# QueensGambit/CrazyAra

Hardware: AMD Instinct MI355X
Metric: nn_evals_per_sec (higher is better)
Workload: dtype f16x3; 1 GPU; crazyhouse RISEv2 19-block (34x8x8 planes -> 5184 policy + value), batch=256, inputs resident in HBM, random-init seeded weights; batch=256, parallelism=replicas x1, precision=float16x3

## Files before the change

crazyara_amd/_capi.py:

```python
from __future__ import annotations

import ctypes as C
import os

_HERE = os.path.dirname(os.path.abspath(__file__))
LIB_PATH = os.path.join(_HERE, "lib", "libcrazyara_hip.so")

c_float_p = C.POINTER(C.c_float)
c_int_p = C.POINTER(C.c_int)

SIGNATURES = {
    "mi_last_error": (C.c_char_p, []),
    "mi_version": (C.c_char_p, []),
    "mi_device_count": (C.c_int, []),
    "mi_host_alloc": (C.c_void_p, [C.c_size_t]),
    "mi_host_free": (None, [C.c_void_p]),
    "mi_net_create": (C.c_void_p, [C.c_char_p, C.c_int, C.c_int, C.c_char_p]),
    "mi_net_destroy": (None, [C.c_void_p]),
    "mi_net_calibrate_int8": (C.c_int, [C.c_char_p, C.c_int, C.c_void_p, C.c_int]),
    "mi_net_has_int8_calibration": (C.c_int, [C.c_char_p]),
    "mi_onnx_to_cranet": (C.c_int, [C.c_char_p, C.c_char_p]),
    "mi_e4m3_from_float": (C.c_int, [C.c_float]),
    "mi_e5m2_from_float": (C.c_int, [C.c_float]),
    "mi_net_design": (C.c_int, [C.c_void_p, c_int_p, c_int_p, c_int_p, c_int_p, c_int_p]),
# ... 1 lines not shown
    "mi_net_flops_per_position": (C.c_double, [C.c_void_p]),
    "mi_net_predict": (C.c_int, [C.c_void_p, C.c_void_p, C.c_void_p, C.c_void_p, C.c_void_p]),
    "mi_net_submit": (C.c_int, [C.c_void_p, C.c_void_p, C.c_void_p, C.c_void_p, C.c_void_p]),
    "mi_net_last_submit_zero_copy": (C.c_int, [C.c_void_p]),
    "mi_net_wait": (C.c_int, [C.c_void_p]),
    "mi_net_device_buffers": (C.c_int, [C.c_void_p] + [C.POINTER(C.c_void_p)] * 5),
    "mi_net_keep_logits": (C.c_int, [C.c_void_p, C.c_int]),
    "mi_net_block_dump": (C.c_void_p, [C.c_void_p, c_int_p]),
    "mi_net_forward_device": (C.c_int, [C.c_void_p]),
    "mi_net_sync": (C.c_int, [C.c_void_p]),
    "mi_net_stream": (C.c_void_p, [C.c_void_p]),
    "mi_net_time_forward": (C.c_int, [C.c_void_p, C.c_int, c_float_p]),
    "mi_net_op_count": (C.c_int, [C.c_void_p]),
    "mi_net_time_ops": (C.c_int, [C.c_void_p, C.c_int, C.POINTER(C.c_char_p), c_float_p]),
    "mi_net_op_kernel": (C.c_char_p, [C.c_void_p, C.c_int]),
    "mi_net_submit_boards": (C.c_int, [C.c_void_p, C.c_void_p, C.c_int, C.c_int, C.c_void_p, C.c_void_p, C.c_void_p]),
    "mi_net_submit_boards_gathered": (C.c_int, [C.c_void_p, C.c_void_p, C.c_int, C.c_int, C.c_void_p, C.c_void_p, C.c_uint, C.c_void_p,
                                                C.c_void_p, C.c_void_p]),
    "mi_net_create_experts": (C.c_void_p, [C.c_char_p, C.c_int, C.c_int, C.c_char_p, C.c_int]),
    "mi_net_num_experts": (C.c_int, [C.c_void_p]),
    "mi_expert_dirs": (C.c_int, [C.c_char_p, C.c_int, C.c_int, C.c_char_p, C.c_int]),
    "mi_net_set_expert_routing": (C.c_int, [C.c_void_p, C.c_int]),
    "mi_net_submit_boards_phases": (C.c_int, [C.c_void_p, C.c_void_p, C.c_int, c_int_p]),
    "mi_net_predict_routed": (C.c_int, [C.c_void_p, C.c_void_p, C.c_void_p, C.c_void_p, C.c_void_p, C.c_void_p]),
    "mi_desc_game_phase": (C.c_int, [C.c_void_p, C.c_int, C.c_int]),
    "mi_pos_create": (C.c_void_p, [C.c_char_p, C.c_int, C.c_char_p]),
    "mi_pos_clone": (C.c_void_p, [C.c_void_p]),
    "mi_pos_destroy": (None, [C.c_void_p]),
    "mi_pos_fen": (C.c_int, [C.c_void_p, C.c_char_p, C.c_int]),
    "mi_pos_side_to_move": (C.c_int, [C.c_void_p]),
# ... 100 lines not shown
```

crazyara_amd/csrc/capi.cpp:

```cpp
#include "../../include/crazyara_hip.h"

#include <hip/hip_runtime.h>

#include <exception>
#include <stdexcept>
#include <string>

#include "capi_common.h"
#include "nn/onnx_import.h"
#include "nn/rise_net.h"

namespace {
thread_local std::string g_err;
template <typename F> int guard(F&& f) { return cra_guard(static_cast<F&&>(f)); }
}

void cra_set_error(const std::string& msg) { g_err = msg; }
const char* cra_get_error() { return g_err.c_str(); }

#include "capi_net.h"

namespace {
cra::RiseNet& plain_net(const mi_net* net, const char* what, const char* why = nullptr) {
    if (!net->plain)
// ... 193 lines not shown
    return guard([&] { net->any->wait(); });
}
void* mi_net_stream(mi_net* net) { return net ? static_cast<void*>(net->any->stream()) : nullptr; }

int mi_net_time_forward(mi_net* net, int iters, float* ms_total) {
    if (!net || !ms_total) { g_err = "null argument"; return 1; }
    return guard([&] { *ms_total = plain_net(net, "a device-resident forward").time_forward(iters); });
}
int mi_net_op_count(const mi_net* net) { return net && net->plain ? net->plain->launches_per_forward() : 0; }
const char* mi_net_op_kernel(const mi_net* net, int op) {
    if (!net || !net->plain || op < 0 || op >= net->plain->launches_per_forward()) { g_err = "mi_net_op_kernel: no such op"; return nullptr; }
    const char* name = nullptr;
    if (guard([&] { name = net->plain->op_kernel(op); })) return nullptr;
    return name;
}
int mi_net_time_ops(mi_net* net, int iters, const char** names, float* ms) {
    if (!net || !ms) { g_err = "null argument"; return 1; }
    return guard([&] {
        cra::RiseNet& plain = plain_net(net, "per-op timing");
        const int n = plain.launches_per_forward();
        for (int i = 0; i < n; ++i) {
            if (names) names[i] = plain.op_name(i);
            ms[i] = 0.f;
        }
        plain.time_ops(iters, ms);
    });
}

}
```

crazyara_amd/csrc/nn/kernels.h:

```cpp
#pragma once
#include <hip/hip_runtime.h>
#include <cstdint>

namespace cra {

typedef _Float16 half_t;

constexpr int kSquares = 64;

inline int64_t packed_weight_elems(int cout_pad, int k_total) { return int64_t(cout_pad) * k_total; }

struct ConvArgs {
    const void* x;
    const void* wpk;
    const void* wpk_lo;
    const float* bias;
    const void* resid;
    void* out;
    int batch;
    int cin;
    int cout_pad;
    int cout_real;
    int cout_ld;
    int ks;
// ... 51 lines not shown
    float w1_inv, w3_scale, w3_inv;
    int tail;
};
static_assert(sizeof(X3TowerBlock) == 96, "the tower kernels index a device array of these");
struct X3TowerArgs {
    const float* x;
    float* y;
    const X3TowerBlock* blocks;
    int nblocks;
    int batch;
    int p8;
    int ks;
    int symmetric;
    int no_tail;
    int no_quad;
};
void launch_tower_x3(const X3TowerArgs& a, hipStream_t s);
const char* tower_x3_kernel_name(const X3TowerArgs& a);
void launch_tower_x3_tail(const X3TowerArgs& a, hipStream_t s);
void init_x3_tail_kernel_attributes();
void launch_tower_x3_quad(const X3TowerArgs& a, hipStream_t s);
void init_x3_quad_kernel_attributes();
bool block_x3w_supports(int C, int ks);
void launch_block_x3w(const BlockArgs& a, hipStream_t s);
void init_x3_wblock_kernel_attributes();
void launch_se_gate_w(const float* pool, float* gate, int kind, const float* w1t, const float* w2t, const float* b1, int batch, int C, hipStream_t s);
constexpr int kX3WSplitMaxG = 8;
struct X3WSplitArgs {
    BlockArgs blk;
    const float* x_parts;
    float* y_parts;
    int gin, G;
    int stream_in;
};
int x3w_split_chunks(int cop_pad);
int x3w_split_shares(int cop_pad, int boards, int cu_count);
void launch_block_x3w_split(const X3WSplitArgs& a, hipStream_t s);
// ... 225 lines not shown
```

crazyara_amd/csrc/nn/precision.cpp:

```cpp
#include <cstdlib>
#include <stdexcept>

#include "rise_net.h"

namespace cra {

namespace {
constexpr bool kX3ValueHeadOneLaunch = true;
}

RiseNet::DevSwitches::DevSwitches() {
    if (const char* e = getenv("CRA_X3_CONV_DEV")) conv_dev = atoi(e);
    device_graph = getenv("CRA_DEVICE_GRAPH") != nullptr;
    lane_graph = getenv("CRA_LANE_GRAPH") != nullptr;
    lane_no_graph = getenv("CRA_LANE_NO_GRAPH") != nullptr;
    predict_copy = getenv("CRA_PREDICT_COPY") != nullptr;
    predict_zero_copy = getenv("CRA_PREDICT_ZERO_COPY") != nullptr;
    if (const char* e = getenv("CRA_LANE_LAUNCHES")) lane_launches = e[0];
    lane_sync = getenv("CRA_LANE_SYNC") != nullptr;
    if (const char* e = getenv("CRA_X3_TOWER")) x3_symmetric = e[0] == 's';
    if (const char* e = getenv("CRA_X3_SPLIT_DEV")) x3_split_dev = atoi(e);
    no_small_path = getenv("CRA_NO_SMALL_PATH") != nullptr;
    if (const char* e = getenv("CRA_SMALL_BATCH_CONV_SPLIT")) small_conv_split = atoi(e);
    tower_trace = getenv("CRA_TOWER_TRACE") != nullptr;
    x3_value_one_launch = kX3ValueHeadOneLaunch;
    if (const char* e = getenv("CRA_X3_VALUE_HEAD")) x3_value_one_launch = e[0] == 'o';
    value_head_debug = getenv("CRA_VALUE_HEAD_DEBUG") != nullptr;
    if (const char* e = getenv("CRA_VALUE_HEAD_LDS_PAD")) value_head_lds_pad = atoi(e);
    if (const char* e = getenv("CRA_VALUE_HEAD_VARIANT")) value_head_variant = atoi(e);
    x3_no_head_chain = getenv("CRA_X3_NO_HEAD_CHAIN") != nullptr;
    x3_no_tail = getenv("CRA_X3_NO_TAIL") != nullptr;
    x3_no_quad = getenv("CRA_X3_NO_QUAD") != nullptr;
    small_batch_heads_apart = getenv("CRA_SMALL_BATCH_HEADS_APART") != nullptr;
}

Precision parse_precision(const std::string& precision) {
    Precision v;
    std::string prec = precision;
    auto strip = [&](const std::string& tag) {
        if (prec.size() <= tag.size() || prec.compare(prec.size() - tag.size(), tag.size(), tag) != 0) return false;
        prec.resize(prec.size() - tag.size());
        return true;
    };
    if (strip("-3k")) v.one_launch = false;
    if (strip("-8w")) v.thin_waves = true;
    if (strip("-1wg")) v.board_split = false;
    if (strip("-1b")) v.boards_per_wg = 1;
// ... 33 lines not shown
```

crazyara_amd/csrc/nn/rise_net.h:

```cpp
#pragma once
#include <hip/hip_runtime.h>
#include <memory>
#include <string>
#include <utility>
#include <vector>

#include "board_net.h"
#include "netfile.h"

namespace cra {

uint8_t float_to_e4m3(float v);
uint8_t float_to_e5m2(float v);

struct Precision {
    enum class Mode { Float32, Float16, Float16x3, Float16p8, Fp8, Int8 };
    Mode mode = Mode::Float16;
    bool fused = true;
    bool tower = true;
    bool one_launch = true;
    bool thin_waves = false;
    bool board_split = true;
    bool wblock = false;
    bool wnet = false;
// ... 41 lines not shown
    void run_group(const Group& g);

    std::vector<std::pair<float, float>> calibration_maxima(const float* planes_host, int n_boards);

    void keep_logits(bool on) override;
    void* enable_block_dump(int* n_tiles);
    void dev_launch_op(int op, int iters);
    float* value_head_debug() const { return value_head_dbg_; }
    int dev_screen_prepare();
    long dev_screen_run(int op, int launches, long* words);
    std::string dev_screen_info(int op) const;
    void forward_async();

    int launches_per_forward() const { return launches_; }
    const char* op_name(int i) const;
    const char* op_kernel(int i) const;
    void time_ops(int iters, float* ms);
    float time_forward(int iters);

    struct IoOverride {
        const float* planes = nullptr;
        float* value = nullptr;
        float* probs = nullptr;
        float* aux = nullptr;
    };
    bool last_submit_was_zero_copy() const { return last_zero_copy_; }

private:
    friend class ExpertSet;
    struct ForwardCall {
// ... 23 lines not shown
        bool predict_copy = false;
        bool predict_zero_copy = false;
        char lane_launches = 0;
        bool lane_sync = false;
        bool x3_symmetric = false;
        int x3_split_dev = 0;
        bool no_small_path = false;
        int small_conv_split = 2;
        bool tower_trace = false;
        bool x3_value_one_launch;
        bool value_head_debug = false;
        int value_head_lds_pad = -1;
        int value_head_variant = 0;
        bool x3_no_head_chain = false;
        bool x3_no_tail = false;
        bool x3_no_quad = false;
        bool small_batch_heads_apart = false;
        DevSwitches();
    } dev_;
    float* value_head_dbg_ = nullptr;

    std::string model_file_path_;
    Precision prec_;
    std::vector<std::pair<float, float>> int8_calib_;
    static constexpr int kBoardSplitMaxBatch = 64;
    std::unique_ptr<RiseNet> small_;
    bool owns_stream_ = true;
    int stream_slot_ = -1;
    std::string precision_arg_;
    int cu_count_ = 256;
// ... 14 lines not shown
```

crazyara_amd/csrc/nn/rise_net.hip:

```cpp
#include "rise_net.h"

#include <cmath>
#include <cstdio>
#include <cstring>
#include <fstream>
#include <algorithm>

#include "net_streams.h"
#include "onnx_import.h"
#include "rise_net_impl.h"
#include "../chess/planes_host.h"

namespace cra {

RiseNet::RiseNet(const std::string& model_path, int device_id, int batch_size, const std::string& precision, const RiseNet* parent)
    : BoardNet(device_id), impl_(new Impl) {
    if (batch_size <= 0) throw std::invalid_argument("batch size must be positive");
    precision_arg_ = precision;
    prec_ = parse_precision(precision);
    design_.batch = batch_size;

    std::string dir, file;
    auto ends_with = [&](const char* ext) { const size_t n = strlen(ext); return model_path.size() > n && model_path.compare(model_path.size() - n, n, ext) == 0; };
    if (ends_with(".cranet") || ends_with(".onnx")) {
// ... 244 lines not shown
        case OpKind::X3SplitFinish: return "x3_split_finish";
        case OpKind::HeadsSmall: return "heads_small";
        case OpKind::Attention: return "attention";
        case OpKind::BlockX3W: return "block_x3w";
        case OpKind::NtbX3W: return "ntb_x3w";
        case OpKind::TowerX3W: return "tower_x3w";
        case OpKind::BlockX3WSplit: return "block_x3w_split";
        case OpKind::X3WSplitFinish: return "x3w_split_finish";
    }
    return "?";
}

const char* RiseNet::op_kernel(int i) const {
    const Op& op = impl_->ops.at(i);
    return op.kind == OpKind::TowerX3 ? tower_x3_kernel_name(op.tx) : op_name(i);
}

void RiseNet::time_ops(int iters, float* ms) {
    HIP_CHECK(hipSetDevice(device_));
    hipEvent_t e0, e1;
    HIP_CHECK(hipEventCreate(&e0));
    HIP_CHECK(hipEventCreate(&e1));
    const int n = int(impl_->ops.size());
    for (int it = 0; it < iters; ++it)
        for (int i = 0; i < n; ++i) {
            HIP_CHECK(hipEventRecord(e0, stream_));
            ForwardCall call;
            if (prec_.fp16()) launch_op<half_t>(i, stream_, call); else launch_op<float>(i, stream_, call);
            HIP_CHECK(hipEventRecord(e1, stream_));
            HIP_CHECK(hipEventSynchronize(e1));
// ... 452 lines not shown
```

crazyara_amd/csrc/nn/rise_net_build.hip:

```cpp
#include <algorithm>
#include <cmath>
#include <cstring>
#include <type_traits>

#include "../chess/planes_host.h"
#include "pack.h"
#include "rise_net_impl.h"

namespace cra {

namespace {
enum class Family {
    Tower,
    X3Tower,
    X3Split,
    Fused,
    WBlock,
    WSplit,
    WTower,
    Layers,
    Transformer,
    WNtb
};
struct BlockPlan {
// ... 713 lines not shown
        fin.xs_y = reinterpret_cast<float*>(nxt);
        im.ops.push_back(fin);
    } else {
        Op op;
        op.kind = OpKind::TowerX3;
        op.tx.x = reinterpret_cast<const float*>(cur);
        op.tx.y = reinterpret_cast<float*>(nxt);
        op.tx.blocks = im.upload(x3_blocks);
        op.tx.nblocks = int(x3_blocks.size());
        op.tx.batch = B;
        op.tx.p8 = prec.p8() ? 1 : 0;
        op.tx.ks = x3_run_ks;
        op.tx.symmetric = dev.x3_symmetric ? 1 : 0;
        op.tx.no_tail = dev.x3_no_tail ? 1 : 0;
        op.tx.no_quad = dev.x3_no_quad ? 1 : 0;
        im.ops.push_back(op);
    }
    x3_blocks.clear();
    prod_op = -1;
    std::swap(cur, nxt);
}

template <typename T> void RiseNet::Builder<T>::one_launch_head() {
    const Folded fv = fold_bn(nf, "value_head.body.0", "value_head.body.1");
    const HeadStreams hs = pack_head(fold_bn(nf, "policy_head.body.0", "policy_head.body.1"), fold_bn(nf, "policy_head.body.3", ""), fv, C, cv, cp);
    Op op;
    op.kind = OpKind::Head;
    HeadArgs& h = op.hd;
    h.x = cur;
    h.logits = net.d_logits_;
// ... 245 lines not shown
```

crazyara_amd/csrc/nn/x3.hip:

```cpp
#include "kernels.h"
#include "device_utils.h"
#include "value_head_body.h"
#include "x3_device.h"

#include <algorithm>
#include <cstdlib>
#include <stdexcept>
#include <type_traits>

#ifndef X3_SGB_VALU
#define X3_SGB_VALU 10
#endif

namespace cra {

namespace {

typedef int i32x4_x3 __attribute__((ext_vector_type(4)));
typedef int i32x8_x3 __attribute__((ext_vector_type(8)));
__device__ __forceinline__ uint32_t x3_high_bytes(uint32_t p01, uint32_t p23) {
    return __builtin_amdgcn_perm(p23, p01, 0x07050301u);
}
__device__ __forceinline__ void split4_b8(const float (&v)[4], half4& hi, uint32_t& h8, uint32_t& l8) {
    uint32_t h[2], l[2];
// ... 1962 lines not shown
int block_x3_chunk_channels() { return X3Block::CK; }

void launch_block_x3(const BlockArgs& a, hipStream_t s) {
    hipLaunchKernelGGL(block_x3_kernel, dim3(a.batch), dim3(X3Block::NTHR), X3Block::lds_bytes, s, a);
}
void launch_block_x3_split(const X3SplitArgs& a, hipStream_t s) {
    const int n = a.blk.cop_pad / X3Block::CK;
    if (a.G < 1 || a.G > n || a.G > 16 || a.gin < 1 || a.gin > 16) throw std::invalid_argument("block_x3_split: 1 <= G <= min(chunks, 16), 1 <= gin <= 16");
    hipLaunchKernelGGL(block_x3_split_kernel, dim3(8 * a.G * ((a.batch + 7) / 8)), dim3(X3Block::NTHR), X3Block::lds_bytes, s, a);
}
void launch_x3_split_finish(const float* parts, int gin, float* y, int batch, hipStream_t s) {
    const int n4 = batch * 64 * X3Block::C / 4;
    hipLaunchKernelGGL(x3_split_finish_kernel, dim3(std::min(1024, (n4 + 255) / 256)), dim3(256), 0, s, parts, gin, y, batch);
}
namespace {
enum class X3TowerKernel { P8_5, P8_3, Quad3, Tail5, Tail3, Roles5, Roles3, Symmetric };
X3TowerKernel pick_tower_x3(const X3TowerArgs& a) {
    const bool symmetric = a.symmetric != 0;
    if (a.p8) {
        if (symmetric) throw std::invalid_argument("Precision float16p8 runs the two-role tower only");
        return a.ks == 5 ? X3TowerKernel::P8_5 : X3TowerKernel::P8_3;
    }
    if (!symmetric && !a.no_tail) {
        if (a.ks == 5) return X3TowerKernel::Tail5;
        return a.no_quad ? X3TowerKernel::Tail3 : X3TowerKernel::Quad3;
    }
    if (a.ks == 5) return X3TowerKernel::Roles5;
    return symmetric ? X3TowerKernel::Symmetric : X3TowerKernel::Roles3;
}
}
const char* tower_x3_kernel_name(const X3TowerArgs& a) {
    switch (pick_tower_x3(a)) {
        case X3TowerKernel::P8_5: return "tower_p8_kernel<5>";
        case X3TowerKernel::P8_3: return "tower_p8_kernel<3>";
        case X3TowerKernel::Quad3: return "tower_x3_quad_kernel<3>";
        case X3TowerKernel::Tail5: return "tower_x3_tail_kernel<5>";
        case X3TowerKernel::Tail3: return "tower_x3_tail_kernel<3>";
        case X3TowerKernel::Roles5: return "tower_x3_roles_kernel<5>";
        case X3TowerKernel::Roles3: return "tower_x3_roles_kernel<3>";
        case X3TowerKernel::Symmetric: return "tower_x3_kernel";
    }
    return "?";
}
void launch_tower_x3(const X3TowerArgs& a, hipStream_t s) {
    switch (pick_tower_x3(a)) {
        case X3TowerKernel::P8_5: hipLaunchKernelGGL(tower_p8_kernel<5>, dim3(a.batch), dim3(X3Block::NTHR), X3Block::lds_bytes + 8192, s, a); break;
        case X3TowerKernel::P8_3: hipLaunchKernelGGL(tower_p8_kernel<3>, dim3(a.batch), dim3(X3Block::NTHR), X3Block::lds_bytes, s, a); break;
        case X3TowerKernel::Quad3: launch_tower_x3_quad(a, s); break;
        case X3TowerKernel::Tail5:
        case X3TowerKernel::Tail3: launch_tower_x3_tail(a, s); break;
        case X3TowerKernel::Roles5: hipLaunchKernelGGL(tower_x3_roles_kernel<5>, dim3(a.batch), dim3(X3Block::NTHR), X3Block::lds_bytes + 8192, s, a); break;
        case X3TowerKernel::Roles3: hipLaunchKernelGGL(tower_x3_roles_kernel<3>, dim3(a.batch), dim3(X3Block::NTHR), X3Block::lds_bytes, s, a); break;
        case X3TowerKernel::Symmetric: hipLaunchKernelGGL(tower_x3_kernel, dim3(a.batch), dim3(X3Block::NTHR), X3Block::lds_bytes, s, a); break;
    }
}

}
```

crazyara_amd/csrc/nn/x3_quad.cpp:

```cpp
#include "x3_device.h"
#include "x3_quad.h"

#include <type_traits>

namespace cra {

template <int KS>
__global__ __launch_bounds__(512) void tower_x3_quad_kernel(const X3TowerArgs a) {
    static_assert(KS == 3, "depthwise 3x3 (X3DepthwiseQuad); 5x5 runs stay on tower_x3_tail_kernel");
    constexpr int REC = 256;
    using G = X3Block;
    static_assert(G::NE == 1 && G::T2BUF == 2 && G::CK == 128, "the role kernel uses the NE = 1 tile geometry (two t2 buffers of 128 channels)");
    static_assert(X3Q_T2T_HALVES <= 64 * G::TROW, "t2T of a chunk lies in the [64][TROW] tile's place");
    constexpr int C = G::C, CK = G::CK, XROW = G::XROW, TROW = G::TROW;
    extern __shared__ __attribute__((aligned(16))) char smem[];
    const X3Tiles T = x3_tiles(smem);
    const int b = blockIdx.x;
    const int tid = threadIdx.x, lane = tid & 63, l15 = lane & 15, lg = lane >> 4;
    const int wave = __builtin_amdgcn_readfirstlane(tid >> 6);
    const bool expand_role = wave < 4;
    const int w = wave & 3;
    const uint32_t lane_off = uint32_t(lane) * 16u;
    x3_stage_tile(T, a.x + size_t(b) * 64 * C, nullptr, tid);
    __syncthreads();
    constexpr int EW = 2;
    half8 e_h[EW][2], e_l[EW][2];
    bool first_chunk_requested = false;
    if (expand_role) {
    for (int blk = 0; blk < a.nblocks; ++blk) {
        const X3TowerBlock& d = a.blocks[blk];
        if (blk > 0 && d.se_kind != 0) {
            x3_se_gate_from_mean(d, reinterpret_cast<float*>(T.t2h), tid);
            __syncthreads();
            first_chunk_requested = false;
#pragma unroll
            for (int ne = 0; ne < 2; ++ne) {
#pragma unroll
// ... 62 lines not shown
                if constexpr (HASE) {
#pragma unroll
                    for (int ne = 0; ne < NEE; ++ne)
#pragma unroll
                        for (int h2 = 0; h2 < REC / 256; ++h2)
                            dw_raw[ne][h2] = __builtin_bit_cast(f32x4, __builtin_amdgcn_raw_buffer_load_b128(W.dw, lane_off, uint32_t(e_tile(i, ne) * 16) * uint32_t(REC / 4) + uint32_t(h2) * 1024u, 0));
#pragma unroll
                    for (int ne = 0; ne < NEE; ++ne)
#pragma unroll
                        for (int t = 0; t < 4; ++t) accE[ne][t] = f32x4{0.f, 0.f, 0.f, 0.f};
                    read_step(0); read_step(1); read_step(2);
                }
                if constexpr (HASD) dw.load(my_dws, l15, qo);
                half_t* const t2h = T.t2h + ((i - 1) & 1) * 64 * TROW;
                half_t* const t2l = T.t2l + ((i - 1) & 1) * 64 * TROW;
#pragma unroll
                for (int sl = 0; sl < (ONED ? C / 64 : C / 32); ++sl) {
                    const int dt = sl / 4, ph = sl % 4;
                    if constexpr (HASD) {
                        if (!ONED && sl == 3) dw.load(my_dws + 256, l15, qo);
                    }
                    __builtin_amdgcn_sched_barrier(0);
                    if constexpr (HASE) {
#pragma unroll
                        for (int t = 0; t < 4; ++t) {
                            const int st = sl * 4 + t;
                            if (st + 3 < 4 * (C / 32)) read_step(st + 3);
#pragma unroll
                            for (int ne = 0; ne < NEE; ++ne) {
                                x3_mfma(ring_h[st % 4], e_l[sl % EW][ne], accE[ne][t], !(X3_ABL & 2));
                                x3_mfma(ring_l[st % 4], e_h[sl % EW][ne], accE[ne][t], !(X3_ABL & 2));
                                x3_mfma(ring_h[st % 4], e_h[sl % EW][ne], accE[ne][t], !(X3_ABL & 2));
                            }
// ... 18 lines not shown
                                    *reinterpret_cast<half4*>(t2h + tile * 16 * X3Q_T2T_ROW + sto[t]) = h;
                                    *reinterpret_cast<half4*>(t2l + tile * 16 * X3Q_T2T_ROW + sto[t]) = l;
                                }
                            }
                        }
                    }
                    if constexpr (HASE && HASD) {
#pragma unroll
                        for (int r = 0; r < 12 * NEE; ++r) {
                            __builtin_amdgcn_sched_group_barrier(0x008, 1, 0);
                            __builtin_amdgcn_sched_group_barrier(0x002, ONEE ? 8 : 4, 0);
                        }
                    }
                    __builtin_amdgcn_sched_barrier(0);
                }
                if constexpr (HASE) {
#pragma unroll
                    for (int ne = 0; ne < NEE; ++ne)
#pragma unroll
                        for (int h2 = 0; h2 < REC / 256; ++h2) *reinterpret_cast<f32x4*>(my_dws + ne * REC + h2 * 256 + lane * 4) = dw_raw[ne][h2];
#pragma unroll
                    for (int ne = 0; ne < NEE; ++ne)
#pragma unroll
                        for (int t = 0; t < 4; ++t) accD[ne][t] = accE[ne][t];
                }
            };
            constexpr std::true_type yes{};
            constexpr std::false_type no{};
            auto run = [&](auto hase_c, auto hasd_c, auto onee_c, auto oned_c, int i) {
                const int kk = i - 1;
                X3_STAMP(0);
                interval(hase_c, hasd_c, onee_c, oned_c, i);
                X3_STAMP(3);
                if constexpr (!(X3_ABL & 32)) __syncthreads();
                X3_STAMP(4);
            };
            const int nfull = tail ? n - 1 : n;
            if (nfull == 0) run(yes, no, yes, no, 0);
            else run(yes, no, no, no, 0);
            for (int i = 1; i < nfull; ++i) run(yes, yes, no, no, i);
            if (tail) {
                if (nfull > 0) run(yes, yes, yes, no, n - 1);
                run(no, yes, no, yes, n);
            } else run(no, yes, no, no, n);
            first_chunk_requested = false;
            if (blk + 1 < a.nblocks && a.blocks[blk + 1].se_kind == 0) {
                const X3TowerBlock& dn = a.blocks[blk + 1];
                load_first_chunk(x3_weights(dn.w1pk, dn.w1pk_lo, dn.w3pk, dn.w3pk_lo, dn.dwpk, dn.cop_pad), dn.tail != 0 && dn.cop_pad == CK);
                first_chunk_requested = true;
            }
            __syncthreads();
            { const int kk = n; X3_STAMP(5); }
        }
    }
    } else {
    constexpr int NJ = 4;
    f32x4 accX[NJ][4];
    x3_stream_load<NJ>(accX, a.x + size_t(b) * 64 * C, w * NJ, l15, lg);
    for (int blk = 0; blk < a.nblocks; ++blk) {
        const X3TowerBlock& d = a.blocks[blk];
        if (blk > 0 && d.se_kind != 0) x3_stream_se<NJ>(T, d, accX, reinterpret_cast<float*>(T.t2h), w * NJ, tid);
        const X3Weights W = x3_weights(d.w1pk, d.w1pk_lo, d.w3pk, d.w3pk_lo, d.dwpk, d.cop_pad);
        const int n = W.cop_pad / CK;
        const int nslab3 = W.cop_pad >> 5;
        const bool tail = __builtin_amdgcn_readfirstlane(d.tail) != 0;
// ... 15 lines not shown
                for (int j = 0; j < NJ; ++j) {
                    const uint32_t f = uint32_t(w * NJ + j) * uint32_t(nslab3) + uint32_t(k * (CK / 32) + s2);
                    p_h[s2 % PW][j] = x3_frag(W.w3h, lane_off, f);
                    p_l[s2 % PW][j] = x3_frag(W.w3l, lane_off, f);
                }
            };
            if constexpr (X3_ABL & 16) {
#pragma unroll
                for (int s2 = 0; s2 < PW; ++s2)
#pragma unroll
                    for (int j = 0; j < NJ; ++j) p_h[s2][j] = p_l[s2][j] = *reinterpret_cast<const half8*>(T.xl + lane * 8);
            }
            x3_stream_add_bias<NJ>(accX, d.b3, w * NJ, lg);
#pragma unroll
            for (int s2 = 0; s2 < PW; ++s2) load_p(0, s2);
            if constexpr (!(X3_ABL & 32)) {
                __syncthreads();
                __syncthreads();
            }
            auto project = [&](auto one_c, int kk) {
                constexpr int NS2 = decltype(one_c)::value ? CK / 64 : CK / 32;
                const half_t* const t2h = T.t2h + (kk & 1) * 64 * TROW;
                const half_t* const t2l = T.t2l + (kk & 1) * 64 * TROW;
                const half_t* rd[2][4];
#pragma unroll
                for (int hh = 0; hh < 2; ++hh)
#pragma unroll
                    for (int t = 0; t < 4; ++t) rd[hh][t] = t2h + rdo[hh][t];
                const int to_lo = int(t2l - t2h);
                X3_STAMP(8);
                half8 bh[2][4], bl[2][4];
                auto read_t2 = [&](int s2, half8 (&h)[4], half8 (&l)[4]) {
#pragma unroll
                    for (int t = 0; t < 4; ++t) {
                        if constexpr (X3_ABL & 8) {
                            h[t] = p_h[s2 % PW][0];
                            l[t] = p_l[s2 % PW][0];
                        } else {
                            h[t] = x3q_read_fragment(rd[0][t] + s2 * 32 * X3Q_T2T_ROW, rd[1][t] + s2 * 32 * X3Q_T2T_ROW);
                            l[t] = x3q_read_fragment(rd[0][t] + s2 * 32 * X3Q_T2T_ROW + to_lo, rd[1][t] + s2 * 32 * X3Q_T2T_ROW + to_lo);
                        }
                    }
                };
                read_t2(0, bh[0], bl[0]);
#pragma unroll
                for (int s2 = 0; s2 < NS2; ++s2) {
                    if (s2 + 1 < NS2) read_t2(s2 + 1, bh[(s2 + 1) & 1], bl[(s2 + 1) & 1]);
                    __builtin_amdgcn_sched_barrier(0);
#pragma unroll
                    for (int j = 0; j < NJ; ++j)
#pragma unroll
                        for (int t = 0; t < 4; ++t) x3_mfma(p_l[s2 % PW][j], bh[s2 & 1][t], accX[j][t], !(X3_ABL & 4));
#pragma unroll
                    for (int j = 0; j < NJ; ++j)
#pragma unroll
                        for (int t = 0; t < 4; ++t) x3_mfma(p_h[s2 % PW][j], bl[s2 & 1][t], accX[j][t], !(X3_ABL & 4));
#pragma unroll
                    for (int j = 0; j < NJ; ++j)
#pragma unroll
                        for (int t = 0; t < 4; ++t) x3_mfma(p_h[s2 % PW][j], bh[s2 & 1][t], accX[j][t], !(X3_ABL & 4));
                    if (s2 + PW < NS2) load_p(kk, s2 + PW);
                    else if constexpr (decltype(one_c)::value) load_p(kk, s2 + PW - NS2);
                    else load_p(kk + 1 < n ? kk + 1 : kk, s2 + PW - NS2);
                    if (s2 == 1) X3_STAMP(9);
                    __builtin_amdgcn_sched_barrier(0);
                }
                X3_STAMP(10);
            };
            const int nfull = tail ? n - 1 : n;
            for (int kk = 0; kk < nfull; ++kk) {
                project(std::false_type{}, kk);
                if (kk + 1 < n) {
                    if constexpr (!(X3_ABL & 32)) __syncthreads();
                }
                X3_STAMP(11);
            }
            if (tail) {
                const int kk = n - 1;
                project(std::true_type{}, kk);
                X3_STAMP(11);
            }
            if (blk + 1 < a.nblocks && a.blocks[blk + 1].se_kind == 0) x3_stream_write_tiles<NJ>(T, accX, w * NJ, l15, lg);
            { const int kk = n; X3_STAMP(12); }
            __syncthreads();
            { const int kk = n; X3_STAMP(13); }
        }
    }
    x3_stream_store<NJ>(accX, a.y + size_t(b) * 64 * C, w * NJ, l15, lg);
    }
}

void init_x3_quad_kernel_attributes() {
    (void)hipFuncSetAttribute(reinterpret_cast<const void*>(&tower_x3_quad_kernel<3>), hipFuncAttributeMaxDynamicSharedMemorySize, int(X3Block::lds_bytes));
}
void launch_tower_x3_quad(const X3TowerArgs& a, hipStream_t s) {
    hipLaunchKernelGGL(tower_x3_quad_kernel<3>, dim3(a.batch), dim3(X3Block::NTHR), X3Block::lds_bytes, s, a);
}

}
```

crazyara_amd/neuralnetapi.py:

```python
from __future__ import annotations

import ctypes as C
import os
import sys
from typing import Optional

import numpy as np

from . import _capi

VERSION_SEP_MAJOR = 1000000
VERSION_SEP_MINOR = 1000


def make_version(major: int, minor: int, patch: int = 0) -> int:
    return major * VERSION_SEP_MAJOR + minor * VERSION_SEP_MINOR + patch


class _DevArray:

    def __init__(self, ptr: int, shape, typestr="<f4"):
        self.__cuda_array_interface__ = {"shape": tuple(shape), "typestr": typestr, "data": (int(ptr), False), "version": 2}


# ... 132 lines not shown
        n = self._lib.mi_net_op_count(self._h)
        names = (C.c_char_p * n)()
        ms = (C.c_float * n)()
        if self._lib.mi_net_time_ops(self._h, int(iters), names, ms):
            raise RuntimeError(_capi.last_error())
        return [(names[i].decode(), ms[i] / iters) for i in range(n)]

    def op_kernels(self):
        out = []
        for i in range(self._lib.mi_net_op_count(self._h)):
            name = self._lib.mi_net_op_kernel(self._h, i)
            if name is None:
                raise RuntimeError(_capi.last_error())
            out.append(name.decode())
        return out

    def close(self) -> None:
        if getattr(self, "_h", None):
            self._lib.mi_net_destroy(self._h)
            self._h = None

    def __del__(self):
        try:
            self.close()
        except Exception:
            pass


PHASE_LICHESS, PHASE_MOVECOUNT = 0, 1
ROUTE_PER_BOARD, ROUTE_MAJORITY = 0, 1
# ... 92 lines not shown
```

include/crazyara_hip.h:

```cpp
#ifndef CRAZYARA_HIP_H
#define CRAZYARA_HIP_H

#include <stddef.h>
#include <stdint.h>

#ifdef __cplusplus
extern "C" {
#endif

const char* mi_last_error(void);
const char* mi_version(void);
int mi_device_count(void);

void* mi_host_alloc(size_t bytes);
void mi_host_free(void* p);

typedef struct mi_net mi_net;

mi_net* mi_net_create(const char* model_dir, int device_id, int batch_size, const char* precision);
int mi_net_calibrate_int8(const char* model_dir, int device_id, const float* planes, int n_boards);
int mi_net_has_int8_calibration(const char* model_dir);
void mi_net_destroy(mi_net* net);

int mi_e4m3_from_float(float v);
// ... 10 lines not shown
int mi_net_submit(mi_net* net, const float* in_planes, float* value, float* probs, float* aux);
int mi_net_wait(mi_net* net);
int mi_net_last_submit_zero_copy(const mi_net* net);

int mi_net_device_buffers(mi_net* net, float** d_planes, float** d_value, float** d_probs, float** d_logits, float** d_aux);
int mi_net_keep_logits(mi_net* net, int on);
void* mi_net_block_dump(mi_net* net, int* n_tiles);
int mi_net_forward_device(mi_net* net);
int mi_net_sync(mi_net* net);
void* mi_net_stream(mi_net* net);

int mi_net_time_forward(mi_net* net, int iters, float* ms_total);
int mi_net_op_count(const mi_net* net);
int mi_net_time_ops(mi_net* net, int iters, const char** names, float* ms);
const char* mi_net_op_kernel(const mi_net* net, int op);

typedef struct mi_pos mi_pos;
enum { MI_MODE_CRAZYHOUSE = 0, MI_MODE_CHESS = 1, MI_MODE_LICHESS = 2 };
enum { MI_TERMINAL_LOSS = 0, MI_TERMINAL_DRAW = 1, MI_TERMINAL_WIN = 2, MI_TERMINAL_CUSTOM = 3, MI_TERMINAL_NONE = 4 };

mi_pos* mi_pos_create(const char* fen, int is_chess960, const char* variant);
mi_pos* mi_pos_clone(const mi_pos* pos);
void mi_pos_destroy(mi_pos* pos);
int mi_pos_fen(const mi_pos* pos, char* buf, int cap);
int mi_pos_side_to_move(const mi_pos* pos);
int mi_pos_legal_moves(const mi_pos* pos, uint32_t* moves, int cap);
uint32_t mi_pos_uci_to_move(const mi_pos* pos, const char* uci);
int mi_pos_move_to_uci(const mi_pos* pos, uint32_t move, char* buf, int cap);
int mi_pos_move_to_san(const mi_pos* pos, uint32_t move, char* buf, int cap);
int mi_pos_do_move(mi_pos* pos, uint32_t move);
// ... 164 lines not shown
```

Baseline: 356,200 evals/s.

## Replace workgroup barriers in quad tower kernel with LDS flag-based producer/consumer flow

Adds a FLOW variant of the quad tower kernel in which expand and project waves coordinate through per-wave progress counters in LDS (filled/drained) instead of __syncthreads between intervals. Expand waves wait only until the projection has drained the double-buffered t2 slot from two steps earlier, and projection waves wait until every expand wave has filled the current slot. The goal is to let the two roles run ahead of each other and remove full-workgroup barrier stalls. The cost is spin-polling with s_sleep and a bounded poll budget that falls back to a sticky timeout flag, plus extra LDS and new API hooks to inspect the sync mode and timeout count. It is on by default; CRA_X3_NO_FLOW turns it off.

```diff
diff --git a/crazyara_amd/_capi.py b/crazyara_amd/_capi.py
--- a/crazyara_amd/_capi.py
+++ b/crazyara_amd/_capi.py
@@ -39,6 +39,8 @@
     "mi_net_op_count": (C.c_int, [C.c_void_p]),
     "mi_net_time_ops": (C.c_int, [C.c_void_p, C.c_int, C.POINTER(C.c_char_p), c_float_p]),
     "mi_net_op_kernel": (C.c_char_p, [C.c_void_p, C.c_int]),
+    "mi_net_op_sync": (C.c_char_p, [C.c_void_p, C.c_int]),
+    "mi_net_x3_flow_timeouts": (C.c_long, [C.c_void_p]),
     "mi_net_submit_boards": (C.c_int, [C.c_void_p, C.c_void_p, C.c_int, C.c_int, C.c_void_p, C.c_void_p, C.c_void_p]),
     "mi_net_submit_boards_gathered": (C.c_int, [C.c_void_p, C.c_void_p, C.c_int, C.c_int, C.c_void_p, C.c_void_p, C.c_uint, C.c_void_p,
                                                 C.c_void_p, C.c_void_p]),
diff --git a/crazyara_amd/csrc/capi.cpp b/crazyara_amd/csrc/capi.cpp
--- a/crazyara_amd/csrc/capi.cpp
+++ b/crazyara_amd/csrc/capi.cpp
@@ -231,6 +231,18 @@
     if (guard([&] { name = net->plain->op_kernel(op); })) return nullptr;
     return name;
 }
+const char* mi_net_op_sync(const mi_net* net, int op) {
+    if (!net || !net->plain || op < 0 || op >= net->plain->launches_per_forward()) { g_err = "mi_net_op_sync: no such op"; return nullptr; }
+    const char* name = nullptr;
+    if (guard([&] { name = net->plain->op_sync(op); })) return nullptr;
+    return name;
+}
+long mi_net_x3_flow_timeouts(mi_net* net) {
+    if (!net || !net->plain) { g_err = "mi_net_x3_flow_timeouts: not a plain net"; return -1; }
+    long w = -1;
+    if (guard([&] { w = long(net->plain->x3_flow_timeouts()); })) return -1;
+    return w;
+}
 int mi_net_time_ops(mi_net* net, int iters, const char** names, float* ms) {
     if (!net || !ms) { g_err = "null argument"; return 1; }
     return guard([&] {
diff --git a/crazyara_amd/csrc/nn/kernels.h b/crazyara_amd/csrc/nn/kernels.h
--- a/crazyara_amd/csrc/nn/kernels.h
+++ b/crazyara_amd/csrc/nn/kernels.h
@@ -89,13 +89,16 @@
     int symmetric;
     int no_tail;
     int no_quad;
+    int no_flow;
 };
 void launch_tower_x3(const X3TowerArgs& a, hipStream_t s);
 const char* tower_x3_kernel_name(const X3TowerArgs& a);
+const char* tower_x3_sync_name(const X3TowerArgs& a);
 void launch_tower_x3_tail(const X3TowerArgs& a, hipStream_t s);
 void init_x3_tail_kernel_attributes();
 void launch_tower_x3_quad(const X3TowerArgs& a, hipStream_t s);
 void init_x3_quad_kernel_attributes();
+unsigned x3_flow_timeouts();
 bool block_x3w_supports(int C, int ks);
 void launch_block_x3w(const BlockArgs& a, hipStream_t s);
 void init_x3_wblock_kernel_attributes();
diff --git a/crazyara_amd/csrc/nn/precision.cpp b/crazyara_amd/csrc/nn/precision.cpp
--- a/crazyara_amd/csrc/nn/precision.cpp
+++ b/crazyara_amd/csrc/nn/precision.cpp
@@ -31,6 +31,7 @@
     x3_no_head_chain = getenv("CRA_X3_NO_HEAD_CHAIN") != nullptr;
     x3_no_tail = getenv("CRA_X3_NO_TAIL") != nullptr;
     x3_no_quad = getenv("CRA_X3_NO_QUAD") != nullptr;
+    x3_no_flow = getenv("CRA_X3_NO_FLOW") != nullptr;
     small_batch_heads_apart = getenv("CRA_SMALL_BATCH_HEADS_APART") != nullptr;
 }
 
diff --git a/crazyara_amd/csrc/nn/rise_net.h b/crazyara_amd/csrc/nn/rise_net.h
--- a/crazyara_amd/csrc/nn/rise_net.h
+++ b/crazyara_amd/csrc/nn/rise_net.h
@@ -79,6 +79,8 @@
 
     int launches_per_forward() const { return launches_; }
     const char* op_name(int i) const;
+    const char* op_sync(int i) const;
+    unsigned x3_flow_timeouts();
     const char* op_kernel(int i) const;
     void time_ops(int iters, float* ms);
     float time_forward(int iters);
@@ -132,6 +134,7 @@
         int value_head_variant = 0;
         bool x3_no_head_chain = false;
         bool x3_no_tail = false;
+        bool x3_no_flow = false;
         bool x3_no_quad = false;
         bool small_batch_heads_apart = false;
         DevSwitches();
diff --git a/crazyara_amd/csrc/nn/rise_net.hip b/crazyara_amd/csrc/nn/rise_net.hip
--- a/crazyara_amd/csrc/nn/rise_net.hip
+++ b/crazyara_amd/csrc/nn/rise_net.hip
@@ -282,6 +282,17 @@
 const char* RiseNet::op_kernel(int i) const {
     const Op& op = impl_->ops.at(i);
     return op.kind == OpKind::TowerX3 ? tower_x3_kernel_name(op.tx) : op_name(i);
+}
+
+const char* RiseNet::op_sync(int i) const {
+    const Op& op = impl_->ops.at(i);
+    return op.kind == OpKind::TowerX3 ? tower_x3_sync_name(op.tx) : "";
+}
+
+unsigned RiseNet::x3_flow_timeouts() {
+    HIP_CHECK(hipSetDevice(device_));
+    HIP_CHECK(hipStreamSynchronize(stream_));
+    return cra::x3_flow_timeouts();
 }
 
 void RiseNet::time_ops(int iters, float* ms) {
diff --git a/crazyara_amd/csrc/nn/rise_net_build.hip b/crazyara_amd/csrc/nn/rise_net_build.hip
--- a/crazyara_amd/csrc/nn/rise_net_build.hip
+++ b/crazyara_amd/csrc/nn/rise_net_build.hip
@@ -751,6 +751,7 @@
         op.tx.symmetric = dev.x3_symmetric ? 1 : 0;
         op.tx.no_tail = dev.x3_no_tail ? 1 : 0;
         op.tx.no_quad = dev.x3_no_quad ? 1 : 0;
+        op.tx.no_flow = dev.x3_no_flow ? 1 : 0;
         im.ops.push_back(op);
     }
     x3_blocks.clear();
diff --git a/crazyara_amd/csrc/nn/x3.hip b/crazyara_amd/csrc/nn/x3.hip
--- a/crazyara_amd/csrc/nn/x3.hip
+++ b/crazyara_amd/csrc/nn/x3.hip
@@ -2000,7 +2000,7 @@
     hipLaunchKernelGGL(x3_split_finish_kernel, dim3(std::min(1024, (n4 + 255) / 256)), dim3(256), 0, s, parts, gin, y, batch);
 }
 namespace {
-enum class X3TowerKernel { P8_5, P8_3, Quad3, Tail5, Tail3, Roles5, Roles3, Symmetric };
+enum class X3TowerKernel { P8_5, P8_3, Quad3, Quad3Flow, Tail5, Tail3, Roles5, Roles3, Symmetric };
 X3TowerKernel pick_tower_x3(const X3TowerArgs& a) {
     const bool symmetric = a.symmetric != 0;
     if (a.p8) {
@@ -2009,7 +2009,8 @@
     }
     if (!symmetric && !a.no_tail) {
         if (a.ks == 5) return X3TowerKernel::Tail5;
-        return a.no_quad ? X3TowerKernel::Tail3 : X3TowerKernel::Quad3;
+        if (a.no_quad) return X3TowerKernel::Tail3;
+        return a.no_flow ? X3TowerKernel::Quad3 : X3TowerKernel::Quad3Flow;
     }
     if (a.ks == 5) return X3TowerKernel::Roles5;
     return symmetric ? X3TowerKernel::Symmetric : X3TowerKernel::Roles3;
@@ -2019,7 +2020,8 @@
     switch (pick_tower_x3(a)) {
         case X3TowerKernel::P8_5: return "tower_p8_kernel<5>";
         case X3TowerKernel::P8_3: return "tower_p8_kernel<3>";
-        case X3TowerKernel::Quad3: return "tower_x3_quad_kernel<3>";
+        case X3TowerKernel::Quad3:
+        case X3TowerKernel::Quad3Flow: return "tower_x3_quad_kernel<3>";
         case X3TowerKernel::Tail5: return "tower_x3_tail_kernel<5>";
         case X3TowerKernel::Tail3: return "tower_x3_tail_kernel<3>";
         case X3TowerKernel::Roles5: return "tower_x3_roles_kernel<5>";
@@ -2028,11 +2030,13 @@
     }
     return "?";
 }
+const char* tower_x3_sync_name(const X3TowerArgs& a) { return pick_tower_x3(a) == X3TowerKernel::Quad3Flow ? "flow" : "barrier"; }
 void launch_tower_x3(const X3TowerArgs& a, hipStream_t s) {
     switch (pick_tower_x3(a)) {
         case X3TowerKernel::P8_5: hipLaunchKernelGGL(tower_p8_kernel<5>, dim3(a.batch), dim3(X3Block::NTHR), X3Block::lds_bytes + 8192, s, a); break;
         case X3TowerKernel::P8_3: hipLaunchKernelGGL(tower_p8_kernel<3>, dim3(a.batch), dim3(X3Block::NTHR), X3Block::lds_bytes, s, a); break;
-        case X3TowerKernel::Quad3: launch_tower_x3_quad(a, s); break;
+        case X3TowerKernel::Quad3:
+        case X3TowerKernel::Quad3Flow: launch_tower_x3_quad(a, s); break;
         case X3TowerKernel::Tail5:
         case X3TowerKernel::Tail3: launch_tower_x3_tail(a, s); break;
         case X3TowerKernel::Roles5: hipLaunchKernelGGL(tower_x3_roles_kernel<5>, dim3(a.batch), dim3(X3Block::NTHR), X3Block::lds_bytes + 8192, s, a); break;
diff --git a/crazyara_amd/csrc/nn/x3_flow.h b/crazyara_amd/csrc/nn/x3_flow.h
--- /dev/null
+++ b/crazyara_amd/csrc/nn/x3_flow.h
@@ -0,0 +1,74 @@
+#pragma once
+#include <cstdint>
+
+namespace cra {
+
+constexpr int X3F_WAVES = 4;
+constexpr int X3F_LDS_BYTES = 64;
+constexpr int X3F_FILLED_WORD = 0, X3F_DRAINED_WORD = 8;
+constexpr uint32_t X3F_POLL_BUDGET = 1u << 18;
+constexpr uint32_t X3F_TIMEOUT_EXPAND = 1u, X3F_TIMEOUT_PROJECT = 2u;
+
+constexpr uint32_t x3f_progress(int g) { return uint32_t(g + 1); }
+constexpr uint32_t x3f_filled_target(int g) { return x3f_progress(g); }
+constexpr uint32_t x3f_drained_target(int g) { return g >= 2 ? x3f_progress(g - 2) : 0u; }
+constexpr bool x3f_store_waits(int c) { return c >= 2; }
+constexpr bool x3f_reached(uint32_t slowest, uint32_t target) { return int32_t(slowest - target) >= 0; }
+
+}
+
+#ifdef __HIPCC__
+namespace cra {
+namespace {
+
+struct X3Flow {
+    uint32_t* filled;
+    uint32_t* drained;
+    int g0;
+    uint32_t budget;
+};
+__device__ __forceinline__ X3Flow x3f_init(char* smem_end, int tid) {
+    X3Flow f;
+    f.filled = reinterpret_cast<uint32_t*>(smem_end) + X3F_FILLED_WORD;
+    f.drained = reinterpret_cast<uint32_t*>(smem_end) + X3F_DRAINED_WORD;
+    f.g0 = 0;
+    f.budget = X3F_POLL_BUDGET;
+    if (tid < 16) reinterpret_cast<uint32_t*>(smem_end)[tid] = 0u;
+    return f;
+}
+__device__ __forceinline__ void x3f_signal(uint32_t* words, int w, int g, int lane) {
+    __builtin_amdgcn_sched_barrier(0);
+    __atomic_signal_fence(__ATOMIC_SEQ_CST);
+    if (lane == 0) __hip_atomic_store(words + w, x3f_progress(g), __ATOMIC_RELAXED, __HIP_MEMORY_SCOPE_WORKGROUP);
+    __atomic_signal_fence(__ATOMIC_SEQ_CST);
+    __builtin_amdgcn_sched_barrier(0);
+}
+__device__ __forceinline__ int x3f_poll(const uint32_t* words, int lane) {
+    return int(__hip_atomic_load(words + (lane & 3), __ATOMIC_RELAXED, __HIP_MEMORY_SCOPE_WORKGROUP));
+}
+__device__ __forceinline__ bool x3f_all_reached(int v, uint32_t target) {
+    const uint32_t v0 = uint32_t(__builtin_amdgcn_readlane(v, 0)), v1 = uint32_t(__builtin_amdgcn_readlane(v, 1));
+    const uint32_t v2 = uint32_t(__builtin_amdgcn_readlane(v, 2)), v3 = uint32_t(__builtin_amdgcn_readlane(v, 3));
+    return x3f_reached(v0, target) && x3f_reached(v1, target) && x3f_reached(v2, target) && x3f_reached(v3, target);
+}
+__device__ __forceinline__ void x3f_wait(const uint32_t* words, uint32_t target, int polled, uint32_t& budget, unsigned* sticky, uint32_t bit, int lane) {
+    __builtin_amdgcn_sched_barrier(0);
+    __atomic_signal_fence(__ATOMIC_SEQ_CST);
+    bool there = x3f_all_reached(polled, target);
+    while (!there) {
+        if (budget == 0u) {
+            if (lane == 0) atomicOr(sticky, bit);
+            break;
+        }
+        budget = uint32_t(__builtin_amdgcn_readfirstlane(int(budget))) - 1u;
+        __builtin_amdgcn_s_sleep(1);
+        there = x3f_all_reached(x3f_poll(words, lane), target);
+    }
+    __builtin_amdgcn_fence(__ATOMIC_ACQUIRE, "workgroup", "local");
+    __atomic_signal_fence(__ATOMIC_SEQ_CST);
+    __builtin_amdgcn_sched_barrier(0);
+}
+
+}
+}
+#endif
diff --git a/crazyara_amd/csrc/nn/x3_quad.cpp b/crazyara_amd/csrc/nn/x3_quad.cpp
--- a/crazyara_amd/csrc/nn/x3_quad.cpp
+++ b/crazyara_amd/csrc/nn/x3_quad.cpp
@@ -1,11 +1,16 @@
 #include "x3_device.h"
 #include "x3_quad.h"
-
+#include "x3_flow.h"
+
+#include <stdexcept>
+#include <string>
 #include <type_traits>
 
 namespace cra {
 
-template <int KS>
+__device__ unsigned x3_flow_timeout_word;
+
+template <int KS, bool FLOW>
 __global__ __launch_bounds__(512) void tower_x3_quad_kernel(const X3TowerArgs a) {
     static_assert(KS == 3, "depthwise 3x3 (X3DepthwiseQuad); 5x5 runs stay on tower_x3_tail_kernel");
     constexpr int REC = 256;
@@ -21,6 +26,8 @@
     const bool expand_role = wave < 4;
     const int w = wave & 3;
     const uint32_t lane_off = uint32_t(lane) * 16u;
+    X3Flow fl{};
+    if constexpr (FLOW) fl = x3f_init(smem + X3Block::lds_bytes, tid);
     x3_stage_tile(T, a.x + size_t(b) * 64 * C, nullptr, tid);
     __syncthreads();
     constexpr int EW = 2;
@@ -113,9 +120,19 @@
                 if constexpr (HASD) dw.load(my_dws, l15, qo);
                 half_t* const t2h = T.t2h + ((i - 1) & 1) * 64 * TROW;
                 half_t* const t2l = T.t2l + ((i - 1) & 1) * 64 * TROW;
+                [[maybe_unused]] int drained_polled = 0;
 #pragma unroll
                 for (int sl = 0; sl < (ONED ? C / 64 : C / 32); ++sl) {
                     const int dt = sl / 4, ph = sl % 4;
+                    if constexpr (FLOW && HASD && !(X3_ABL & 32)) {
+                        if (sl == 2) drained_polled = x3f_poll(fl.drained, lane);
+                        if (sl == 3 && x3f_store_waits(i - 1)) {
+                            const int kk = i - 1;
+                            X3_STAMP(3);
+                            x3f_wait(fl.drained, x3f_drained_target(fl.g0 + i - 1), drained_polled, fl.budget, &x3_flow_timeout_word, X3F_TIMEOUT_EXPAND, lane);
+                            X3_STAMP(4);
+                        }
+                    }
                     if constexpr (HASD) {
                         if (!ONED && sl == 3) dw.load(my_dws + 256, l15, qo);
                     }
@@ -164,6 +181,7 @@
                     }
                     __builtin_amdgcn_sched_barrier(0);
                 }
+                if constexpr (FLOW && HASD && !(X3_ABL & 32)) x3f_signal(fl.filled, w, fl.g0 + i - 1, lane);
                 if constexpr (HASE) {
 #pragma unroll
                     for (int ne = 0; ne < NEE; ++ne)
@@ -181,9 +199,11 @@
                 const int kk = i - 1;
                 X3_STAMP(0);
                 interval(hase_c, hasd_c, onee_c, oned_c, i);
-                X3_STAMP(3);
-                if constexpr (!(X3_ABL & 32)) __syncthreads();
-                X3_STAMP(4);
+                if constexpr (!FLOW) {
+                    X3_STAMP(3);
+                    if constexpr (!(X3_ABL & 32)) __syncthreads();
+                    X3_STAMP(4);
+                }
             };
             const int nfull = tail ? n - 1 : n;
             if (nfull == 0) run(yes, no, yes, no, 0);
@@ -199,6 +219,7 @@
                 load_first_chunk(x3_weights(dn.w1pk, dn.w1pk_lo, dn.w3pk, dn.w3pk_lo, dn.dwpk, dn.cop_pad), dn.tail != 0 && dn.cop_pad == CK);
                 first_chunk_requested = true;
             }
+            if constexpr (FLOW) fl.g0 += n;
             __syncthreads();
             { const int kk = n; X3_STAMP(5); }
         }
@@ -244,7 +265,7 @@
             x3_stream_add_bias<NJ>(accX, d.b3, w * NJ, lg);
 #pragma unroll
             for (int s2 = 0; s2 < PW; ++s2) load_p(0, s2);
-            if constexpr (!(X3_ABL & 32)) {
+            if constexpr (!FLOW && !(X3_ABL & 32)) {
                 __syncthreads();
                 __syncthreads();
             }
@@ -258,6 +279,11 @@
 #pragma unroll
                     for (int t = 0; t < 4; ++t) rd[hh][t] = t2h + rdo[hh][t];
                 const int to_lo = int(t2l - t2h);
+                if constexpr (FLOW && !(X3_ABL & 32)) {
+                    X3_STAMP(3);
+                    x3f_wait(fl.filled, x3f_filled_target(fl.g0 + kk), x3f_poll(fl.filled, lane), fl.budget, &x3_flow_timeout_word, X3F_TIMEOUT_PROJECT, lane);
+                    X3_STAMP(4);
+                }
                 X3_STAMP(8);
                 half8 bh[2][4], bl[2][4];
                 auto read_t2 = [&](int s2, half8 (&h)[4], half8 (&l)[4]) {
@@ -276,6 +302,9 @@
 #pragma unroll
                 for (int s2 = 0; s2 < NS2; ++s2) {
                     if (s2 + 1 < NS2) read_t2(s2 + 1, bh[(s2 + 1) & 1], bl[(s2 + 1) & 1]);
+                    if constexpr (FLOW && !(X3_ABL & 32)) {
+                        if (s2 == NS2 - 1) x3f_signal(fl.drained, w, fl.g0 + kk, lane);
+                    }
                     __builtin_amdgcn_sched_barrier(0);
 #pragma unroll
                     for (int j = 0; j < NJ; ++j)
@@ -301,7 +330,7 @@
             for (int kk = 0; kk < nfull; ++kk) {
                 project(std::false_type{}, kk);
                 if (kk + 1 < n) {
-                    if constexpr (!(X3_ABL & 32)) __syncthreads();
+                    if constexpr (!FLOW && !(X3_ABL & 32)) __syncthreads();
                 }
                 X3_STAMP(11);
             }
@@ -312,6 +341,7 @@
             }
             if (blk + 1 < a.nblocks && a.blocks[blk + 1].se_kind == 0) x3_stream_write_tiles<NJ>(T, accX, w * NJ, l15, lg);
             { const int kk = n; X3_STAMP(12); }
+            if constexpr (FLOW) fl.g0 += n;
             __syncthreads();
             { const int kk = n; X3_STAMP(13); }
         }
@@ -320,11 +350,21 @@
     }
 }
 
+static_assert(X3Block::lds_bytes % 16 == 0 && X3Block::lds_bytes + X3F_LDS_BYTES <= 160 * 1024, "the counters lie behind the depthwise records");
 void init_x3_quad_kernel_attributes() {
-    (void)hipFuncSetAttribute(reinterpret_cast<const void*>(&tower_x3_quad_kernel<3>), hipFuncAttributeMaxDynamicSharedMemorySize, int(X3Block::lds_bytes));
+    (void)hipFuncSetAttribute(reinterpret_cast<const void*>(&tower_x3_quad_kernel<3, false>), hipFuncAttributeMaxDynamicSharedMemorySize, int(X3Block::lds_bytes));
+    (void)hipFuncSetAttribute(reinterpret_cast<const void*>(&tower_x3_quad_kernel<3, true>), hipFuncAttributeMaxDynamicSharedMemorySize,
+                              int(X3Block::lds_bytes + X3F_LDS_BYTES));
 }
 void launch_tower_x3_quad(const X3TowerArgs& a, hipStream_t s) {
-    hipLaunchKernelGGL(tower_x3_quad_kernel<3>, dim3(a.batch), dim3(X3Block::NTHR), X3Block::lds_bytes, s, a);
-}
-
-}
+    if (a.no_flow) hipLaunchKernelGGL((tower_x3_quad_kernel<3, false>), dim3(a.batch), dim3(X3Block::NTHR), X3Block::lds_bytes, s, a);
+    else hipLaunchKernelGGL((tower_x3_quad_kernel<3, true>), dim3(a.batch), dim3(X3Block::NTHR), X3Block::lds_bytes + X3F_LDS_BYTES, s, a);
+}
+unsigned x3_flow_timeouts() {
+    unsigned w = 0;
+    const hipError_t e = hipMemcpyFromSymbol(&w, HIP_SYMBOL(x3_flow_timeout_word), sizeof(w));
+    if (e != hipSuccess) throw std::runtime_error(std::string("x3_flow_timeouts: ") + hipGetErrorString(e));
+    return w;
+}
+
+}
diff --git a/crazyara_amd/neuralnetapi.py b/crazyara_amd/neuralnetapi.py
--- a/crazyara_amd/neuralnetapi.py
+++ b/crazyara_amd/neuralnetapi.py
@@ -170,6 +170,21 @@
                 raise RuntimeError(_capi.last_error())
             out.append(name.decode())
         return out
+
+    def op_syncs(self):
+        out = []
+        for i in range(self._lib.mi_net_op_count(self._h)):
+            name = self._lib.mi_net_op_sync(self._h, i)
+            if name is None:
+                raise RuntimeError(_capi.last_error())
+            out.append(name.decode())
+        return out
+
+    def x3_flow_timeouts(self) -> int:
+        w = self._lib.mi_net_x3_flow_timeouts(self._h)
+        if w < 0:
+            raise RuntimeError(_capi.last_error())
+        return int(w)
 
     def close(self) -> None:
         if getattr(self, "_h", None):
diff --git a/include/crazyara_hip.h b/include/crazyara_hip.h
--- a/include/crazyara_hip.h
+++ b/include/crazyara_hip.h
@@ -48,6 +48,8 @@
 int mi_net_op_count(const mi_net* net);
 int mi_net_time_ops(mi_net* net, int iters, const char** names, float* ms);
 const char* mi_net_op_kernel(const mi_net* net, int op);
+const char* mi_net_op_sync(const mi_net* net, int op);
+long mi_net_x3_flow_timeouts(mi_net* net);
 
 typedef struct mi_pos mi_pos;
 enum { MI_MODE_CRAZYHOUSE = 0, MI_MODE_CHESS = 1, MI_MODE_LICHESS = 2 };
```

Result: no change. 354,900 evals/s (-0.4%).
